# h33p/ofps

Hardware: AMD Instinct MI355X
Metric: Mvectors/s, 1080p 16x16 blocks +-16 full-search SAD (higher is better)
Workload: dtype u8

## Files before the change

### ofps_amd/csrc/sad_qpel.hip

```cpp
#include "common.hpp"

namespace {

struct QpelParams {
    const uint8_t* prev_base;
    const uint8_t* cur_base;
    size_t prev_pitch, cur_pitch;
    int W, H, stride;
    int nbx, nby, B, R;
    long long total;
    float nx, ny;
    float4* out_entries;
    const int* in_best;
    int* out_best;
};

__host__ __device__ constexpr int q_iw(int B) { return B + 6; }
__host__ __device__ constexpr int q_hw(int B) { return B + 1; }
__host__ __device__ constexpr int q_ps(int B) { return (B + 4 + 3) & ~3; }
__host__ __device__ constexpr int q_rows(int B) { return 2 * B + 3; }
__host__ __device__ constexpr int q_off_b1(int B) { return (q_iw(B) * q_iw(B) + 3) & ~3; }
__host__ __device__ constexpr int q_off_hg(int B) { return q_off_b1(B) + ((q_iw(B) * q_hw(B) * 2 + 3) & ~3); }
__host__ __device__ constexpr int q_off_cur(int B) { return q_off_hg(B) + q_rows(B) * 2 * q_ps(B); }
__host__ __device__ constexpr int q_wave_bytes(int B) { return (q_off_cur(B) + ((B * B + 3) & ~3) + 15) & ~15; }
static_assert(q_wave_bytes(64) <= 64 * 1024, "the generic form keeps one wave's planes in the default LDS allocation");

__device__ __forceinline__ void wave_sync() {
    __builtin_amdgcn_fence(__ATOMIC_RELEASE, "wavefront");
    __builtin_amdgcn_wave_barrier();
    __builtin_amdgcn_fence(__ATOMIC_ACQUIRE, "wavefront");
}

__device__ __forceinline__ unsigned long long shfl_xor_u64(unsigned long long v, int mask) {
    unsigned lo = (unsigned)v, hi = (unsigned)(v >> 32);
    lo = __shfl_xor(lo, mask, 64);
    hi = __shfl_xor(hi, mask, 64);
    return ((unsigned long long)hi << 32) | lo;
}

__device__ __forceinline__ int clampi(int v, int lo, int hi) { return v < lo ? lo : (v > hi ? hi : v); }
__device__ __forceinline__ uint8_t clip255(int v) { return (uint8_t)clampi(v, 0, 255); }

template <typename T>
__device__ __forceinline__ int tap6(const T* s, int step) {
    return (int)s[0] - 5 * (int)s[step] + 20 * (int)s[2 * step] + 20 * (int)s[3 * step] - 5 * (int)s[4 * step] + (int)s[5 * step];
}

__device__ __forceinline__ void phase_offsets(int fx, int fy, int& pox, int& poy, int& qox, int& qoy) {
    const bool ox = fx & 1, oy = fy & 1;
    if (!ox && !oy) { pox = qox = fx >> 1; poy = qoy = fy >> 1; }
    else if (ox && !oy) { pox = (fx - 1) >> 1; qox = (fx + 1) >> 1; poy = qoy = fy >> 1; }
    else if (!ox) { pox = qox = fx >> 1; poy = (fy - 1) >> 1; qoy = (fy + 1) >> 1; }
    else {
        const int xa = (fx - 1) >> 1, ya = (fy - 1) >> 1;
        if ((xa + ya) & 1) { pox = xa; poy = ya; qox = xa + 1; qoy = ya + 1; }
        else { pox = xa + 1; poy = ya; qox = xa; qoy = ya + 1; }
    }
}

template <int BT, int WAVES>
__global__ __launch_bounds__(64 * WAVES) void sad_qpel_kernel(const QpelParams p) {
    extern __shared__ __attribute__((aligned(16))) uint8_t q_lds[];
    const int B = BT ? BT : p.B;
    const int wave = __builtin_amdgcn_readfirstlane(threadIdx.x >> 6);
    const int lane = threadIdx.x & 63;
    const long long k = (long long)blockIdx.x * WAVES + wave;
    if (k >= p.total) return;
    const int per_pair = p.nbx * p.nby;
    const int pair = (int)(k / per_pair);
    const int rem = (int)(k - (long long)pair * per_pair);
    const int by = rem / p.nbx, bx = rem - by * p.nbx;
    const int x0 = bx * B, y0 = by * B;
    const uint8_t* __restrict__ prev = p.prev_base + (size_t)pair * p.prev_pitch;
    const uint8_t* __restrict__ cur = p.cur_base + (size_t)pair * p.cur_pitch;
    const int dx = __builtin_amdgcn_readfirstlane(p.in_best[3 * k + 0]);
    const int dy = __builtin_amdgcn_readfirstlane(p.in_best[3 * k + 1]);

    uint8_t* win = q_lds + (size_t)wave * q_wave_bytes(B);
    int16_t* b1 = reinterpret_cast<int16_t*>(win + q_off_b1(B));
    uint8_t* hg = win + q_off_hg(B);
    uint8_t* cl = win + q_off_cur(B);
    const int IW = q_iw(B), HW = q_hw(B), PS = q_ps(B);

    for (int i = lane; i < IW * IW; i += 64) {
        const int wy = i / IW, wx = i - wy * IW;
        const int gx = clampi(x0 + dx - 3 + wx, 0, p.W - 1), gy = clampi(y0 + dy - 3 + wy, 0, p.H - 1);
        win[i] = prev[(size_t)gy * p.stride + gx];
    }
    if constexpr (BT != 0) {
        constexpr int BW = BT / 4;
        for (int i = lane; i < BT * BW; i += 64) {
            const int y = i / BW, q = i - y * BW;
            reinterpret_cast<uint32_t*>(cl)[i] = *reinterpret_cast<const uint32_t*>(cur + (size_t)(y0 + y) * p.stride + x0 + 4 * q);
        }
    } else {
        for (int i = lane; i < B * B; i += 64) {
            const int y = i / B, x = i - y * B;
            cl[i] = cur[(size_t)(y0 + y) * p.stride + x0 + x];
        }
    }
    wave_sync();

    for (int i = lane; i < IW * HW; i += 64) {
        const int wy = i / HW, hx = i - wy * HW;
        b1[i] = (int16_t)tap6(win + wy * IW + hx, 1);
    }
    wave_sync();

    {
        const int NE = B + 2, NO = B + 1;
        auto at = [&](int Y2, int X2) -> uint8_t& { return hg[(Y2 * 2 + (X2 & 1)) * PS + (X2 >> 1)]; };
        for (int i = lane; i < NE * NE; i += 64) {
            const int iy = i / NE, ix = i - iy * NE;
            at(2 * iy, 2 * ix) = win[(iy + 2) * IW + ix + 2];
        }
        for (int i = lane; i < NE * NO; i += 64) {
            const int iy = i / NO, ix = i - iy * NO;
            at(2 * iy, 2 * ix + 1) = clip255(((int)b1[(iy + 2) * HW + ix] + 16) >> 5);
        }
        for (int i = lane; i < NO * NE; i += 64) {
            const int iy = i / NE, ix = i - iy * NE;
            at(2 * iy + 1, 2 * ix) = clip255((tap6(win + iy * IW + ix + 2, IW) + 16) >> 5);
        }
        for (int i = lane; i < NO * NO; i += 64) {
            const int iy = i / NO, ix = i - iy * NO;
            at(2 * iy + 1, 2 * ix + 1) = clip255((tap6(b1 + iy * HW + ix, HW) + 512) >> 10);
        }
    }
    wave_sync();

    const int cand = lane < 49 ? lane : 48;
    const int fy = cand / 7 - 3, fx = cand - (cand / 7) * 7 - 3;
    int pox, poy, qox, qoy;
    phase_offsets(fx, fy, pox, poy, qox, qoy);
    const int prow = ((poy + 2) * 2 + (pox & 1)) * PS, qrow = ((qoy + 2) * 2 + (qox & 1)) * PS;
    const int pk = (pox + 2) >> 1, qk = (qox + 2) >> 1;
    uint32_t sad = 0;
    if constexpr (BT != 0) {
        constexpr int BW = BT / 4;
        const uint32_t* pp = reinterpret_cast<const uint32_t*>(hg + prow);
        const uint32_t* qp = reinterpret_cast<const uint32_t*>(hg + qrow);
        const uint32_t* cp = reinterpret_cast<const uint32_t*>(cl);
        const int RS = PS;
#pragma unroll
        for (int y = 0; y < BT; ++y) {
            uint32_t a[BW + 1], b[BW + 1];
#pragma unroll
            for (int g = 0; g <= BW; ++g) { a[g] = pp[y * RS + g]; b[g] = qp[y * RS + g]; }
#pragma unroll
            for (int g = 0; g < BW; ++g) {
                const uint32_t pa = __builtin_amdgcn_alignbyte(a[g + 1], a[g], (uint32_t)pk);
                const uint32_t qb = __builtin_amdgcn_alignbyte(b[g + 1], b[g], (uint32_t)qk);
                const uint32_t avg = (pa | qb) - (((pa ^ qb) >> 1) & 0x7F7F7F7Fu);
                sad = __builtin_amdgcn_sad_u8(avg, cp[y * BW + g], sad);
            }
        }
    } else {
        const uint8_t* pp = hg + prow + pk;
        const uint8_t* qp = hg + qrow + qk;
        for (int y = 0; y < B; ++y)
            for (int x = 0; x < B; ++x) {
                const int s = ((int)pp[y * 4 * PS + x] + (int)qp[y * 4 * PS + x] + 1) >> 1;
                const int d = (int)cl[y * B + x] - s;
                sad += (uint32_t)(d < 0 ? -d : d);
            }
    }

    const int Dx = 4 * dx + fx, Dy = 4 * dy + fy;
    const bool valid = lane < 49 && 4 * x0 + Dx >= 0 && 4 * (x0 + B - 1) + Dx <= 4 * (p.W - 1) && 4 * y0 + Dy >= 0 &&
                       4 * (y0 + B - 1) + Dy <= 4 * (p.H - 1);
    const int bias = 4 * p.R + 3;
    unsigned long long best = ~0ull;
    if (valid)
        best = ((unsigned long long)sad << 40) | ((unsigned long long)(uint32_t)(Dx * Dx + Dy * Dy) << 20) |
               ((unsigned long long)(uint32_t)(Dy + bias) << 10) | (unsigned long long)(uint32_t)(Dx + bias);
#pragma unroll
    for (int m = 32; m >= 1; m >>= 1) {
        const unsigned long long o = shfl_xor_u64(best, m);
        best = o < best ? o : best;
    }
    if (lane == 0) {
        const int bsad = (int)(best >> 40);
        const int bDy = (int)((best >> 10) & 1023) - bias, bDx = (int)(best & 1023) - bias;
        const int cx = x0 + B / 2, cy = y0 + B / 2;
        float4 e;
        e.x = ((float)(4 * cx + bDx) * 0.25f) * p.nx;
        e.y = ((float)(4 * cy + bDy) * 0.25f) * p.ny;
        e.z = ((float)bDx / 4.0f) * (-p.nx);
        e.w = ((float)bDy / 4.0f) * (-p.ny);
        p.out_entries[k] = e;
        if (p.out_best) {
            p.out_best[3 * k + 0] = bDx;
            p.out_best[3 * k + 1] = bDy;
            p.out_best[3 * k + 2] = bsad;
        }
    }
}

template <int BT, int WAVES>
void launch_qpel(const QpelParams& p, hipStream_t s) {
    const unsigned nwg = (unsigned)((p.total + WAVES - 1) / WAVES);
    hipLaunchKernelGGL((sad_qpel_kernel<BT, WAVES>), dim3(nwg), dim3(64 * WAVES), (size_t)WAVES * q_wave_bytes(p.B), s, p);
}

}

namespace ofps {
int sad_qpel_refine_device(ofps_hip_ctx* ctx, const uint8_t* prev_base, size_t prev_pitch, const uint8_t* cur_base, size_t cur_pitch,
                           int pairs, int W, int H, int stride, int block, int range, void* d_entries, const void* d_in_best,
                           void* d_out_best) {
    OFPS_REQUIRE(ctx, block >= 1 && block <= 64 && range >= 0 && range <= kSadHierMaxReach, "sad_qpel: block=%d range=%d outside [1,64]/[0,127]",
                 block, range);
    OFPS_REQUIRE(ctx, d_entries && d_in_best, "sad_qpel: null device pointer");
    QpelParams p{};
    p.prev_base = prev_base; p.cur_base = cur_base;
    p.prev_pitch = prev_pitch; p.cur_pitch = cur_pitch;
    p.W = W; p.H = H; p.stride = stride;
    p.nbx = W / block; p.nby = H / block; p.B = block; p.R = range;
    p.total = (long long)p.nbx * p.nby * pairs;
    p.nx = 1.0f / (float)W; p.ny = 1.0f / (float)H;
    p.out_entries = static_cast<float4*>(d_entries);
    p.in_best = static_cast<const int*>(d_in_best);
    p.out_best = static_cast<int*>(d_out_best);
    if (p.total <= 0) return OFPS_HIP_OK;
    OFPS_REQUIRE(ctx, p.total < (1ll << 31), "sad_qpel: grid too large");
    if (block == 16) launch_qpel<16, 4>(p, ctx->stream);
    else if (block == 8) launch_qpel<8, 4>(p, ctx->stream);
    else launch_qpel<0, 1>(p, ctx->stream);
    OFPS_HIP_TRY(ctx, hipGetLastError());
    return OFPS_HIP_OK;
}
}

extern "C" {

int ofps_hip_set_sad_motion_scale(ofps_hip_ctx* ctx, int scale) {
    if (!ctx) return OFPS_HIP_EINVAL;
    OFPS_REQUIRE(ctx, scale == 1 || scale == 4, "set_sad_motion_scale: %d is not 1 (full-pel) or 4 (quarter-pel)", scale);
    ctx->opt.sad_motion_scale = scale;
    return OFPS_HIP_OK;
}

int ofps_hip_get_sad_motion_scale(ofps_hip_ctx* ctx) { return ctx ? ctx->opt.sad_motion_scale : OFPS_HIP_EINVAL; }

}
```

Baseline: 518.0.

## Vectorize quarter-pel interpolation with packed 16-bit taps and dword window loads

For compile-time block sizes, the byte-wise window fetch and scalar six-tap filters are replaced with dword-aligned global loads using alignbyte, and with packed u16x2 six-tap horizontal and vertical filters. These write half-pel planes as 4-byte words into a new LDS layout. The change also adds a min-waves launch bound and reduces the SAD row unroll to 4 to lower register pressure. It aims to cut LDS byte traffic and ALU work in the interpolation stage, which runs on every qpel refinement. In exchange the indexing is more complex, and the 16-bit intermediates carry a risk of overflow or wrap in the centre-tap path.

After: 519.9, median of 6. No clear change (+0.4%).

```diff
diff --git a/ofps_amd/csrc/sad_qpel.hip b/ofps_amd/csrc/sad_qpel.hip
--- a/ofps_amd/csrc/sad_qpel.hip
+++ b/ofps_amd/csrc/sad_qpel.hip
@@ -46,6 +46,30 @@
     return (int)s[0] - 5 * (int)s[step] + 20 * (int)s[2 * step] + 20 * (int)s[3 * step] - 5 * (int)s[4 * step] + (int)s[5 * step];
 }
 
+__host__ __device__ constexpr int qp_off_b1(int B) { return (q_iw(B) * q_ps(B) + 7) & ~7; }
+__host__ __device__ constexpr int qp_off_hg(int B) { return qp_off_b1(B) + ((q_iw(B) * q_ps(B) * 2 + 7) & ~7); }
+__host__ __device__ constexpr int qp_off_cur(int B) { return (qp_off_hg(B) + q_rows(B) * 2 * q_ps(B) + 15) & ~15; }
+__host__ __device__ constexpr int qp_wave_bytes(int B) { return (qp_off_cur(B) + B * B + 15) & ~15; }
+
+using u16x2 = unsigned short __attribute__((ext_vector_type(2)));
+using i16x2 = short __attribute__((ext_vector_type(2)));
+__device__ __forceinline__ u16x2 as_pk(uint32_t v) { return __builtin_bit_cast(u16x2, v); }
+
+__device__ __forceinline__ u16x2 tap6_pk(u16x2 s0, u16x2 s1, u16x2 s2, u16x2 s3, u16x2 s4, u16x2 s5) {
+    const u16x2 m5 = {65531, 65531}, k20 = {20, 20};
+    return (s0 + s5) + (s1 + s4) * m5 + (s2 + s3) * k20;
+}
+
+__device__ __forceinline__ uint32_t round5_pk(u16x2 v) {
+    const u16x2 r = {16, 16};
+    i16x2 t = __builtin_bit_cast(i16x2, v + r) >> 5;
+    const i16x2 lo = {0, 0}, hi = {255, 255};
+    t = __builtin_elementwise_min(__builtin_elementwise_max(t, lo), hi);
+    return __builtin_bit_cast(uint32_t, t);
+}
+
+__device__ __forceinline__ uint32_t pack4(uint32_t a, uint32_t b) { return __builtin_amdgcn_perm(b, a, 0x06040200u); }
+
 __device__ __forceinline__ void phase_offsets(int fx, int fy, int& pox, int& poy, int& qox, int& qoy) {
     const bool ox = fx & 1, oy = fy & 1;
     if (!ox && !oy) { pox = qox = fx >> 1; poy = qoy = fy >> 1; }
@@ -59,7 +83,7 @@
 }
 
 template <int BT, int WAVES>
-__global__ __launch_bounds__(64 * WAVES) void sad_qpel_kernel(const QpelParams p) {
+__global__ __launch_bounds__(64 * WAVES, BT ? 4 : 1) void sad_qpel_kernel(const QpelParams p) {
     extern __shared__ __attribute__((aligned(16))) uint8_t q_lds[];
     const int B = BT ? BT : p.B;
     const int wave = __builtin_amdgcn_readfirstlane(threadIdx.x >> 6);
@@ -76,38 +100,119 @@
     const int dx = __builtin_amdgcn_readfirstlane(p.in_best[3 * k + 0]);
     const int dy = __builtin_amdgcn_readfirstlane(p.in_best[3 * k + 1]);
 
-    uint8_t* win = q_lds + (size_t)wave * q_wave_bytes(B);
-    int16_t* b1 = reinterpret_cast<int16_t*>(win + q_off_b1(B));
-    uint8_t* hg = win + q_off_hg(B);
-    uint8_t* cl = win + q_off_cur(B);
+    uint8_t* win = q_lds + (size_t)wave * (BT ? qp_wave_bytes(BT) : q_wave_bytes(B));
+    uint8_t* hg = win + (BT ? qp_off_hg(BT) : q_off_hg(B));
+    uint8_t* cl = win + (BT ? qp_off_cur(BT) : q_off_cur(B));
     const int IW = q_iw(B), HW = q_hw(B), PS = q_ps(B);
 
-    for (int i = lane; i < IW * IW; i += 64) {
-        const int wy = i / IW, wx = i - wy * IW;
-        const int gx = clampi(x0 + dx - 3 + wx, 0, p.W - 1), gy = clampi(y0 + dy - 3 + wy, 0, p.H - 1);
-        win[i] = prev[(size_t)gy * p.stride + gx];
-    }
     if constexpr (BT != 0) {
-        constexpr int BW = BT / 4;
+        constexpr int BW = BT / 4, NG = q_ps(BT) / 4, ROWS = BT + 6;
+        constexpr int DI = 64 / NG, DG = 64 - DI * NG;
         for (int i = lane; i < BT * BW; i += 64) {
             const int y = i / BW, q = i - y * BW;
             reinterpret_cast<uint32_t*>(cl)[i] = *reinterpret_cast<const uint32_t*>(cur + (size_t)(y0 + y) * p.stride + x0 + 4 * q);
         }
+        uint8_t* aw = win;
+        uint8_t* b1p = win + qp_off_b1(BT);
+        const int xs = x0 + dx - 3, ys = y0 + dy - 3;
+        const bool inside = xs >= 0 && xs + ROWS - 1 <= p.W - 1;
+        const uint32_t ph = (uint32_t)(xs & 3);
+        const int ndw = ((xs & 3) + ROWS + 3) >> 2;
+        {
+            int wy = lane / NG, g = lane - (lane / NG) * NG;
+            for (; wy < ROWS; wy += DI) {
+                const uint8_t* row = prev + (size_t)clampi(ys + wy, 0, p.H - 1) * p.stride;
+                uint32_t w0, w1, w2;
+                if (inside) {
+                    const uint32_t* rd = reinterpret_cast<const uint32_t*>(row) + (xs >> 2);
+                    const int last = ndw - 1;
+                    const uint32_t d0 = rd[g < last ? g : last], d1 = rd[g + 1 < last ? g + 1 : last], d2 = rd[g + 2 < last ? g + 2 : last];
+                    w0 = __builtin_amdgcn_alignbyte(d1, d0, ph);
+                    w1 = __builtin_amdgcn_alignbyte(d2, d1, ph);
+                    w2 = __builtin_amdgcn_alignbyte(0u, d2, ph);
+                } else {
+                    w0 = w1 = 0;
+#pragma unroll
+                    for (int t = 0; t < 4; ++t) {
+                        w0 |= (uint32_t)row[clampi(xs + 4 * g + t, 0, p.W - 1)] << (8 * t);
+                        w1 |= (uint32_t)row[clampi(xs + 4 * g + 4 + t, 0, p.W - 1)] << (8 * t);
+                    }
+                    w2 = row[clampi(xs + 4 * g + 8, 0, p.W - 1)];
+                }
+                u16x2 q[8];
+#pragma unroll
+                for (int t = 0; t < 4; ++t) {
+                    const uint32_t sel = 0x0c000c00u | ((uint32_t)(t + 1) << 16) | (uint32_t)t;
+                    q[t] = as_pk(__builtin_amdgcn_perm(w1, w0, sel));
+                    q[t + 4] = as_pk(__builtin_amdgcn_perm(w2, w1, sel));
+                }
+                const u16x2 s01 = tap6_pk(q[0], q[1], q[2], q[3], q[4], q[5]);
+                const u16x2 s23 = tap6_pk(q[2], q[3], q[4], q[5], q[6], q[7]);
+                const uint32_t mid = __builtin_amdgcn_alignbyte(w1, w0, 2u);
+                *reinterpret_cast<uint2*>(b1p + (wy * NG + g) * 8) = make_uint2(__builtin_bit_cast(uint32_t, s01), __builtin_bit_cast(uint32_t, s23));
+                *reinterpret_cast<uint32_t*>(aw + (wy * NG + g) * 4) = mid;
+                if (wy >= 2 && wy < BT + 4) {
+                    uint8_t* grow = hg + (wy - 2) * 4 * PS + 4 * g;
+                    *reinterpret_cast<uint32_t*>(grow) = mid;
+                    *reinterpret_cast<uint32_t*>(grow + PS) = pack4(round5_pk(s01), round5_pk(s23));
+                }
+                g += DG;
+                if (g >= NG) { g -= NG; ++wy; }
+            }
+        }
+        wave_sync();
+
+        {
+            int iy = lane / NG, g = lane - (lane / NG) * NG;
+            for (; iy <= BT; iy += DI) {
+                u16x2 lo[6], hi[6];
+                u16x2 c01[6], c23[6];
+#pragma unroll
+                for (int t = 0; t < 6; ++t) {
+                    const uint32_t r = *reinterpret_cast<const uint32_t*>(aw + ((iy + t) * NG + g) * 4);
+                    lo[t] = as_pk(__builtin_amdgcn_perm(0u, r, 0x0c010c00u));
+                    hi[t] = as_pk(__builtin_amdgcn_perm(0u, r, 0x0c030c02u));
+                    const uint2 c = *reinterpret_cast<const uint2*>(b1p + ((iy + t) * NG + g) * 8);
+                    c01[t] = as_pk(c.x);
+                    c23[t] = as_pk(c.y);
+                }
+                uint8_t* hrow = hg + (2 * iy + 1) * 2 * PS + 4 * g;
+                *reinterpret_cast<uint32_t*>(hrow) = pack4(round5_pk(tap6_pk(lo[0], lo[1], lo[2], lo[3], lo[4], lo[5])),
+                                                           round5_pk(tap6_pk(hi[0], hi[1], hi[2], hi[3], hi[4], hi[5])));
+                const i16x2 a01 = __builtin_bit_cast(i16x2, c01[0] + c01[5]), b01 = __builtin_bit_cast(i16x2, c01[1] + c01[4]),
+                            d01 = __builtin_bit_cast(i16x2, c01[2] + c01[3]);
+                const i16x2 a23 = __builtin_bit_cast(i16x2, c23[0] + c23[5]), b23 = __builtin_bit_cast(i16x2, c23[1] + c23[4]),
+                            d23 = __builtin_bit_cast(i16x2, c23[2] + c23[3]);
+                const int j0 = ((int)a01.x - 5 * (int)b01.x + 20 * (int)d01.x + 512) >> 10;
+                const int j1 = ((int)a01.y - 5 * (int)b01.y + 20 * (int)d01.y + 512) >> 10;
+                const int j2 = ((int)a23.x - 5 * (int)b23.x + 20 * (int)d23.x + 512) >> 10;
+                const int j3 = ((int)a23.y - 5 * (int)b23.y + 20 * (int)d23.y + 512) >> 10;
+                *reinterpret_cast<uint32_t*>(hrow + PS) = pack4((uint32_t)clampi(j0, 0, 255) | ((uint32_t)clampi(j1, 0, 255) << 16),
+                                                                (uint32_t)clampi(j2, 0, 255) | ((uint32_t)clampi(j3, 0, 255) << 16));
+                g += DG;
+                if (g >= NG) { g -= NG; ++iy; }
+            }
+        }
+        wave_sync();
     } else {
+        int16_t* b1 = reinterpret_cast<int16_t*>(win + q_off_b1(B));
+        for (int i = lane; i < IW * IW; i += 64) {
+            const int wy = i / IW, wx = i - wy * IW;
+            const int gx = clampi(x0 + dx - 3 + wx, 0, p.W - 1), gy = clampi(y0 + dy - 3 + wy, 0, p.H - 1);
+            win[i] = prev[(size_t)gy * p.stride + gx];
+        }
         for (int i = lane; i < B * B; i += 64) {
             const int y = i / B, x = i - y * B;
             cl[i] = cur[(size_t)(y0 + y) * p.stride + x0 + x];
         }
-    }
-    wave_sync();
-
-    for (int i = lane; i < IW * HW; i += 64) {
-        const int wy = i / HW, hx = i - wy * HW;
-        b1[i] = (int16_t)tap6(win + wy * IW + hx, 1);
-    }
-    wave_sync();
-
-    {
+        wave_sync();
+
+        for (int i = lane; i < IW * HW; i += 64) {
+            const int wy = i / HW, hx = i - wy * HW;
+            b1[i] = (int16_t)tap6(win + wy * IW + hx, 1);
+        }
+        wave_sync();
+
         const int NE = B + 2, NO = B + 1;
         auto at = [&](int Y2, int X2) -> uint8_t& { return hg[(Y2 * 2 + (X2 & 1)) * PS + (X2 >> 1)]; };
         for (int i = lane; i < NE * NE; i += 64) {
@@ -126,8 +231,8 @@
             const int iy = i / NO, ix = i - iy * NO;
             at(2 * iy + 1, 2 * ix + 1) = clip255((tap6(b1 + iy * HW + ix, HW) + 512) >> 10);
         }
-    }
-    wave_sync();
+        wave_sync();
+    }
 
     const int cand = lane < 49 ? lane : 48;
     const int fy = cand / 7 - 3, fx = cand - (cand / 7) * 7 - 3;
@@ -142,7 +247,7 @@
         const uint32_t* qp = reinterpret_cast<const uint32_t*>(hg + qrow);
         const uint32_t* cp = reinterpret_cast<const uint32_t*>(cl);
         const int RS = PS;
-#pragma unroll
+#pragma unroll 4
         for (int y = 0; y < BT; ++y) {
             uint32_t a[BW + 1], b[BW + 1];
 #pragma unroll
@@ -200,7 +305,7 @@
 template <int BT, int WAVES>
 void launch_qpel(const QpelParams& p, hipStream_t s) {
     const unsigned nwg = (unsigned)((p.total + WAVES - 1) / WAVES);
-    hipLaunchKernelGGL((sad_qpel_kernel<BT, WAVES>), dim3(nwg), dim3(64 * WAVES), (size_t)WAVES * q_wave_bytes(p.B), s, p);
+    hipLaunchKernelGGL((sad_qpel_kernel<BT, WAVES>), dim3(nwg), dim3(64 * WAVES), (size_t)WAVES * (BT ? qp_wave_bytes(BT) : q_wave_bytes(p.B)), s, p);
 }
 
 }
```
